# RicherMans/PLDA

Measured on AMD Instinct MI355X. Metric: PLDA LLR trials/sec, higher is better.
Workload: dtype f32; 1 GPU; C2: 100k i-vectors, featdim 200, 5k speakers; 100k x 100k trials, n = 1; fit 10 EM iters; D_eff=200; enrol_models=100000, test_vectors=100000, parallelism=one GPU, score_dtype=f32 (fp64 bias terms, fp32 MFMA contraction), fit_dtype=f64

## Files before the change

### plda_amd/csrc/common.hpp

```cpp
#pragma once

#include <hip/hip_runtime.h>

#include <cstdint>
#include <cstdio>
#include <mutex>
#include <string>
#include <atomic>
#include <vector>

#include "../../include/plda_hip.h"
#include "layout.hpp"

#ifndef PLDA_DIAG
#define PLDA_DIAG 0
#endif

namespace plda {

extern std::atomic<int64_t> g_device_bytes;
extern std::atomic<int64_t> g_device_bytes_peak;
extern std::atomic<int> g_scratch_poison;
extern thread_local hipStream_t g_call_stream;
constexpr size_t POISON_TAIL = (size_t)64 << 10;
// ... 18 lines not shown
}

struct DevBuf {
  void *p = nullptr;
  size_t cap = 0;
  size_t held = 0;
  DevBuf() = default;
  DevBuf(const DevBuf &) = delete;
  DevBuf &operator=(const DevBuf &) = delete;
  ~DevBuf() { release(); }
  hipError_t reserve(size_t bytes) {
    if (bytes <= cap) return hipSuccess;
    release();
    size_t want = bytes + bytes / 8 + 256, total = want + alloc_extra();
    hipError_t e = hipMalloc(&p, total);
    if (e != hipSuccess) { p = nullptr; return e; }
    cap = want; held = total;
    e = alloc_done(p, total);
    if (e != hipSuccess) release();
    return e;
  }
  void release() { free_counted(p, held); p = nullptr; cap = 0; held = 0; }
  template <typename T> T *as() const { return reinterpret_cast<T *>(p); }
};

struct Tmp {
  void *p = nullptr;
  size_t held = 0;
  Tmp() = default;
  Tmp(const Tmp &) = delete;
  Tmp &operator=(const Tmp &) = delete;
  ~Tmp() { free_counted(p, held); }
  hipError_t alloc(size_t bytes) {
    free_counted(p, held); p = nullptr; held = 0;
    const size_t total = (bytes ? bytes : 8) + alloc_extra();
    hipError_t e = hipMalloc(&p, total);
    if (e != hipSuccess) { p = nullptr; return e; }
    held = total;
    e = alloc_done(p, total);
    if (e != hipSuccess) { free_counted(p, held); p = nullptr; held = 0; }
    return e;
  }
  template <typename T> T *as() { return reinterpret_cast<T *>(p); }
};

}

namespace plda { struct HostPipe; }

namespace plda {
constexpr int CS_MAX = 64;
constexpr int CS_NMAX = 4095;
struct CountSet { int G = 0; int32_t vals[CS_MAX] = {}; };
struct Bt4Table { int btM = -1, btN = -1, colwalk = 0; DevBuf tab; int qbase[8] = {}, qlen[8] = {}; uint64_t used = 0; };
}

struct SyrkChunk { const double *rows; int nrows; int pad; double c1, c2; };

struct plda_handle {
  std::recursive_mutex mu;
  int device = 0;
  hipStream_t own_stream = nullptr;
  hipStream_t stream = nullptr;
  std::string err;

  bool fitted = false;
  int Dout = 0, Din = 0;
  std::vector<double> h_mean, h_transform, h_psi, h_offset;
  plda::DevBuf d_mean, d_transform, d_psi, d_offset;
  void *pin_model = nullptr;
  size_t pin_model_cap = 0;

  int64_t fit_K = 0;
  int fit_D = 0;
  plda::DevBuf f_means, f_counts, f_scatter, f_sum, f_W, f_B;
  plda::DevBuf fit_flag;
  plda::DevBuf fit_sort;
  plda::DevBuf fit_offsets;
  plda::DevBuf fit_hist;
  plda::DevBuf fit_roww;
  plda::DevBuf fit_mu;
  plda::DevBuf fit_csum;
  plda::DevBuf em_rows;
  plda::DevBuf em_mats;
  plda::DevBuf grp_pos, grp_uniq;
  double fit_ms[4] = {0, 0, 0, 0};
  hipEvent_t fit_ev[3] = {nullptr, nullptr, nullptr};
  int *fit_dbad = nullptr;
  double fit_t0 = 0.0;

  bool lda_fitted = false;
  int lda_solver = 0, lda_D = 0, lda_rank = 0;
  int64_t lda_K = 0;
  plda::DevBuf l_means, l_priors, l_xbar, l_scalings, l_coef, l_intercept, l_evr;
  plda::DevBuf lda_work;

  plda::HostPipe *hostpipe = nullptr;
  plda::DevBuf hio_O[2];
  int host_variant = 0;

  uint64_t model_epoch = 0;
  struct OneTrial { uint64_t epoch = ~0ull; int n = 0, D = 0; double logterm = 0.0; std::vector<double> c, ivar, ipsi1; } one;

  void *one_host = nullptr, *one_dev = nullptr;
  size_t one_cap = 0;

  plda::DevBuf s_Apk, s_Bpk, s_rbias, s_rscale, s_cbias, s_rpair, s_cpair;
// ... 376 lines not shown
```

### plda_amd/csrc/score.hip

```cpp
#include "common.hpp"
#include <atomic>
#include <chrono>
#include <cstring>

#include <algorithm>

namespace plda {

typedef float f32x4 __attribute__((ext_vector_type(4)));
typedef float f32x16 __attribute__((ext_vector_type(16)));

#define GLOBAL_AS __attribute__((address_space(1)))
#define LDS_AS __attribute__((address_space(3)))

__device__ __forceinline__ void llr_coef(double n, double psi, double &c, double &var) {
  const double den = n * psi + 1.0;
  c = n * psi / den;
  var = 1.0 + psi / den;
}

__global__ void enrol_bias_kernel(const double *__restrict__ U, const int32_t *__restrict__ n_arr,
                                  int n_uniform, const double *__restrict__ psi, int D, int64_t M,
                                  const double *__restrict__ zmean, const double *__restrict__ zstd,
                                  float *__restrict__ rbias, float *__restrict__ rscale) {
  const int lane = threadIdx.x & 63;
  const int64_t row = (int64_t)blockIdx.x * (blockDim.x >> 6) + (threadIdx.x >> 6);
  if (row >= M) return;
  const double n = n_arr ? (double)n_arr[row] : (double)n_uniform;
  const double *u = U + row * (int64_t)D;
  double acc = 0.0;
  for (int d = lane; d < D; d += 64) {
    double c, var;
    const double p = psi[d];
    llr_coef(n, p, c, var);
    const double cu = c * u[d];
    acc += log(var) - log(1.0 + p) + cu * cu / var;
  }
  for (int o = 32; o > 0; o >>= 1) acc += __shfl_xor(acc, o);
  if (lane == 0) {
    double r = -0.5 * acc, sc = 1.0;
    if (zmean && zstd) {
      const double sd = zstd[row];
      if (sd != 0.0) { sc = 1.0 / sd; r = (r - zmean[row]) * sc; }
    }
    rbias[row] = (float)r;
    if (rscale) rscale[row] = (float)sc;
  }
}

__device__ __forceinline__ void count_coef(const double *__restrict__ psi, int D, int n, double *__restrict__ coef ) {
  __shared__ double red[256];
  double acc = 0.0;
  for (int d = threadIdx.x; d < D; d += 256) {
    double c, var;
    const double p = psi[d];
// ... 56 lines not shown
                                                   float *__restrict__ P) {
  __shared__ float tile[32][65];
  const int64_t row0 = (int64_t)blockIdx.x * 64;
  const int k0 = blockIdx.y * 32;
  const int t = threadIdx.x;
  {
    const int c = t & 31;
    const int k = k0 + c;
    const bool second = (MODE == 1 || MODE == 3) && k >= Dp;
    const int d = second ? k - Dp : k;
    const bool dvalid = d < D && k < ((MODE == 1 || MODE == 3) ? 2 * Dp : Dp);
    const double p = dvalid ? psi[d] : 0.0;
#pragma unroll
    for (int pass = 0; pass < 8; ++pass) {
      const int r = (t >> 5) + pass * 8;
      const int64_t row = row0 + r;
      float val = 0.f;
      if (dvalid && row < R) {
        const double x = X[row * (int64_t)D + d];
        if (MODE == 0 || MODE == 1) {
          const double n = n_arr ? (double)n_arr[row] : (double)n_uniform;
          double cc, var;
          llr_coef(n, p, cc, var);
          double v = second ? -0.5 * (1.0 / var - 1.0 / (1.0 + p)) : cc * x / var;
          if (rs) v *= (double)rs[row];
          val = (float)v;
        } else {
          val = (float)(second ? x * x : x);
        }
      }
      tile[c][r] = val;
    }
  }
  __syncthreads();
  {
    const int r = t & 63;
#pragma unroll
    for (int pass = 0; pass < 2; ++pass) {
      const int q = (t >> 6) + pass * 4;
      const int kq = (k0 >> 2) + q;
      if (kq < KQ) {
        f32x4 v;
        v.x = tile[4 * q + 0][r];
        v.y = tile[4 * q + 1][r];
        v.z = tile[4 * q + 2][r];
        v.w = tile[4 * q + 3][r];
        reinterpret_cast<f32x4 *>(P)[(int64_t)kq * Rpad + row0 + r] = v;
      }
    }
  }
}

template <int SIDE, int RW>
__device__ __forceinline__ void prep_side_body(const int block, const double *__restrict__ X, const double *__restrict__ w, const double *__restrict__ Lptr,
                                               int n_uniform, const double *__restrict__ psi, int D, int64_t R, int64_t Rpad, int KQ,
                                               const double *__restrict__ zmean, const double *__restrict__ zstd,
                                               float *__restrict__ P, float *__restrict__ bias, float *__restrict__ rscale,
                                               float2 *__restrict__ pair) {
  constexpr int RPB = 4 * RW;
  __shared__ float tile[2][64][RPB + 1];
  const int lane = threadIdx.x & 63, wave = threadIdx.x >> 6;
  const int64_t row0 = (int64_t)block * RPB;
  const int64_t wrow0 = row0 + wave * RW;
  const int nchunk = (KQ * 4 + 63) >> 6;
  const bool zn = SIDE == 0 && zmean && zstd;
  float rsf[RW];
#pragma unroll
  for (int j = 0; j < RW; ++j) {
    rsf[j] = 1.f;
    if (zn && wrow0 + j < R) { const double sd = zstd[wrow0 + j]; rsf[j] = (float)(sd != 0.0 ? 1.0 / sd : 1.0); }
  }
  constexpr int PF = RW == 16 ? 1 : 4;
  double acc[RW], xc[PF][RW], xn[PF][RW];
#pragma unroll
  for (int j = 0; j < RW; ++j) acc[j] = 0.0;
  auto fetch = [&](int c, double (&x)[RW]) {
    const int d = c * 64 + lane;
#pragma unroll
    for (int j = 0; j < RW; ++j) {
      const int64_t row = wrow0 + j;
      x[j] = (c < nchunk && d < D && row < R) ? X[row * (int64_t)D + d] : 0.0;
    }
  };
  auto chunk = [&](int c, const double (&x)[RW]) {
    const int d = c * 64 + lane;
    const bool dv = d < D;
    const double wd = dv ? w[d] : 0.0;
    double cc = 0.0, var = 1.0;
    if (SIDE == 0 && dv) llr_coef((double)n_uniform, psi[d], cc, var);
    float(*const tl)[RPB + 1] = tile[c & 1];
#pragma unroll
    for (int j = 0; j < RW; ++j) {
      const double xv = x[j];
      float val = 0.f;
      if (dv && wrow0 + j < R) {
        acc[j] += wd * xv * xv;
        if (SIDE == 0) {
          double v = cc * xv / var;
          if (zn) v *= (double)rsf[j];
          val = (float)v;
        } else {
          val = (float)xv;
        }
      }
      tl[lane][wave * RW + j] = val;
    }
    __syncthreads();
    {
      const int r = threadIdx.x % RPB;
#pragma unroll
      for (int pass = 0; pass < RPB / 16; ++pass) {
        const int q = threadIdx.x / RPB + pass * (256 / RPB);
        const int kq = c * 16 + q;
        if (kq < KQ) {
          f32x4 v;
          v.x = tl[4 * q + 0][r];
          v.y = tl[4 * q + 1][r];
          v.z = tl[4 * q + 2][r];
          v.w = tl[4 * q + 3][r];
          reinterpret_cast<f32x4 *>(P)[(int64_t)kq * Rpad + row0 + r] = v;
        }
      }
    }
  };
#pragma unroll
  for (int k = 0; k < PF; ++k) fetch(k, xn[k]);
  for (int c0 = 0; c0 < nchunk; c0 += PF) {
#pragma unroll
    for (int k = 0; k < PF; ++k)
#pragma unroll
      for (int j = 0; j < RW; ++j) xc[k][j] = xn[k][j];
    if (c0 + PF < nchunk) {
#pragma unroll
      for (int k = 0; k < PF; ++k) fetch(c0 + PF + k, xn[k]);
    }
#pragma unroll
    for (int k = 0; k < PF; ++k)
      if (c0 + k < nchunk) chunk(c0 + k, xc[k]);
  }
  const double Lc = SIDE == 0 ? *Lptr : 0.0;
#pragma unroll
  for (int j = 0; j < RW; ++j) {
    double a = acc[j];
    for (int o = 32; o > 0; o >>= 1) a += __shfl_xor(a, o);
    const int64_t row = wrow0 + j;
    if (lane == 0 && row < R) {
      double r = -0.5 * (a + Lc), sc = 1.0;
      if (zn) {
        const double sd = zstd[row];
        if (sd != 0.0) { sc = 1.0 / sd; r = (r - zmean[row]) * sc; }
      }
      bias[row] = (float)r;
      if (SIDE == 0) { rscale[row] = (float)sc; pair[row] = make_float2((float)r, (float)sc); }
      else pair[row] = make_float2(1.f, (float)r);
    }
  }
}

template <int SIDE, int RW>
__global__ __launch_bounds__(256) void prep_side_kernel(const double *__restrict__ X, const double *__restrict__ w, const double *__restrict__ Lptr,
                                                        int n_uniform, const double *__restrict__ psi, int D, int64_t R, int64_t Rpad, int KQ,
                                                        const double *__restrict__ zmean, const double *__restrict__ zstd,
                                                        float *__restrict__ P, float *__restrict__ bias, float *__restrict__ rscale,
                                                        float2 *__restrict__ pair) {
  prep_side_body<SIDE, RW>((int)blockIdx.x, X, w, Lptr, n_uniform, psi, D, R, Rpad, KQ, zmean, zstd, P, bias, rscale, pair);
}
struct PrepSideArgs { const double *X; const double *w; int64_t R, Rpad; float *P; float *bias; float2 *pair; };
__global__ __launch_bounds__(256) void prep_both_kernel(const PrepSideArgs a, const PrepSideArgs b, int blocksA, const double *__restrict__ Lptr, int n_uniform,
                                                        const double *__restrict__ psi, int D, int KQ, const double *__restrict__ zmean,
                                                        const double *__restrict__ zstd, float *__restrict__ rscale) {
  if ((int)blockIdx.x < blocksA)
    prep_side_body<0, 4>((int)blockIdx.x, a.X, a.w, Lptr, n_uniform, psi, D, a.R, a.Rpad, KQ, zmean, zstd, a.P, a.bias, rscale, a.pair);
  else
    prep_side_body<1, 4>((int)blockIdx.x - blocksA, b.X, b.w, Lptr, 0, psi, D, b.R, b.Rpad, KQ, nullptr, nullptr, b.P, b.bias, nullptr, b.pair);
}

struct CountSetDev { int G; int overflow; int32_t vals[CS_MAX]; };

__global__ void count_presence_kernel(const int32_t *__restrict__ n, int64_t M, unsigned char *__restrict__ present ,
                                      int *__restrict__ flags) {
  for (int64_t i = (int64_t)blockIdx.x * blockDim.x + threadIdx.x; i < M; i += (int64_t)gridDim.x * blockDim.x) {
    const int v = n[i];
    if (v >= 1 && v <= CS_NMAX) present[v] = 1;
    else flags[0] = 1;
  }
}

__global__ __launch_bounds__(256) void count_compact_kernel(const unsigned char *__restrict__ present, const int *__restrict__ flags,
                                                            CountSetDev *__restrict__ out) {
  __shared__ unsigned char pr[CS_NMAX + 1];
  for (int i = threadIdx.x; i <= CS_NMAX; i += 256) pr[i] = present[i];
  __syncthreads();
  if (threadIdx.x >= 64) return;
  const int lane = threadIdx.x;
  int cnt = 0;
  for (int k = 0; k < 64; ++k) cnt += pr[lane * 64 + k] ? 1 : 0;
  int incl = cnt;
  for (int o = 1; o < 64; o <<= 1) { const int t = __shfl_up(incl, o); if (lane >= o) incl += t; }
  const int total = __shfl(incl, 63);
  int pos = incl - cnt;
  for (int k = 0; k < 64; ++k)
    if (pr[lane * 64 + k]) { if (pos < CS_MAX) out->vals[pos] = lane * 64 + k; ++pos; }
  if (lane == 0) { out->G = total; out->overflow = (flags[0] != 0 || total > CS_MAX) ? 1 : 0; }
}

constexpr int64_t CS_ONE_WG = 131072;
struct CountSetHost { CountSetDev set; int seq; };
__global__ __launch_bounds__(1024) void count_set_one_wg_kernel(const int32_t *__restrict__ n, int M, int seq, CountSetHost *__restrict__ out ) {
  __shared__ unsigned char pr[CS_NMAX + 1];
  __shared__ int bad;
  for (int i = threadIdx.x; i <= CS_NMAX; i += 1024) pr[i] = 0;
  if (threadIdx.x == 0) bad = 0;
  __syncthreads();
  for (int i0 = 0; i0 < M; i0 += 4096) {
    int v[4];
#pragma unroll
    for (int u = 0; u < 4; ++u) { const int i = i0 + u * 1024 + (int)threadIdx.x; v[u] = i < M ? n[i] : -1; }
#pragma unroll
    for (int u = 0; u < 4; ++u) {
      if (v[u] >= 1 && v[u] <= CS_NMAX) pr[v[u]] = 1;
      else if (i0 + u * 1024 + (int)threadIdx.x < M) bad = 1;
    }
  }
  __syncthreads();
  if (threadIdx.x >= 64) return;
  const int lane = threadIdx.x;
  int cnt = 0;
// ... 687 lines not shown
        unsigned long long *p = dbg + (((size_t)tseq * 16 + 15) * 8 + wave) * 8;
        p[6] = t_e0; p[7] = t_e1;
      }
    }
    ++tseq;
    c_slot = c_slot == 2 ? 0 : c_slot + 1;
    r0 = c_slot == 0 ? q_r0[0] : (c_slot == 1 ? q_r0[1] : q_r0[2]);
    c0 = c_slot == 0 ? q_c0[0] : (c_slot == 1 ? q_c0[1] : q_c0[2]);
    have = (c_slot == 0 ? q_ok[0] : (c_slot == 1 ? q_ok[1] : q_ok[2])) != 0;
  }
  __builtin_amdgcn_s_waitcnt(0x0070);
  if (CLK && threadIdx.x == 0) {
    const unsigned long long c1 = __builtin_amdgcn_s_memtime(), r1 = __builtin_amdgcn_s_memrealtime();
    unsigned long long *p = dbg + 8 + 4 * (size_t)blockIdx.x;
    p[0] = c1 - clk_c0; p[1] = clk_r0; p[2] = r1; p[3] = (unsigned long long)tseq;
    if (blockIdx.x == 0) { dbg[0] = c1 - clk_c0; dbg[1] = r1 - clk_r0; dbg[2] = (unsigned long long)tseq; }
  }
}
#undef BT2_STEP_LAST
#undef BT2_STEP_SECOND
#undef BT2_STEP_FIRST
#undef BT2_STEP_ODD
#undef BT2_XYC
#undef BT2_LOAD
#undef BT2_MFMA8
#undef BT2_MFMA2
#undef BT2_SB

template <typename I = int64_t>
__device__ __host__ inline I bt4_queue_patches(int x, int pM, int pN, int colwalk) {
  if (colwalk) {
    const I rest = (I)pM * (pN % 8);
    return (I)pM * (pN / 8) + (x < rest ? (rest - x + 7) / 8 : 0);
  }
  const I np = (I)pM * pN;
  return x < np ? (np - x + 7) / 8 : 0;
}
template <typename I>
__device__ __host__ inline void bt4_patch(int x, I k, int pM, int pN, int colwalk, int &pm, int &pn) {
  if (colwalk) {
    const I whole = (I)pM * (pN / 8);
    if (k < whole) { pn = x + 8 * (int)(k / pM); pm = (int)(k % pM); }
    else { const int r = pN % 8; const I q = x + 8 * (k - whole); pm = (int)(q / r); pn = (pN / 8) * 8 + (int)(q % r); }
  } else { const I p = x + 8 * k; pm = (int)(p / pN); pn = (int)(p % pN); }
}
#pragma clang diagnostic push
#pragma clang diagnostic ignored "-Wuninitialized"
#pragma clang diagnostic ignored "-Wsometimes-uninitialized"
#pragma clang diagnostic ignored "-Wconditional-uninitialized"
#include "score_bt4.inc"
#pragma clang diagnostic pop
#include "score_bf16x3.inc"

__global__ __launch_bounds__(64) void bt4_table_kernel(int2 *__restrict__ tab, int btM, int btN, int pM, int pN, int colwalk, const Bt4Queues qs) {
  const int x = blockIdx.x, lane = threadIdx.x;
  int off = BT4_QHDR + qs.qbase[x];
  if (lane == 0) tab[x] = make_int2(off, qs.qlen[x]);
  const int64_t nq = bt4_queue_patches(x, pM, pN, colwalk);
  for (int64_t k = 0; k < nq; ++k) {
    int pm, pn;
    bt4_patch(x, k, pM, pN, colwalk, pm, pn);
    const int tm = pm * BPR + lane / BPC, tn = pn * BPC + lane % BPC;
    const bool ok = lane < BPR * BPC && tm < btM && tn < btN;
    const unsigned long long mask = __ballot(ok);
    if (ok) tab[off + __popcll(mask & ((1ull << lane) - 1ull))] = make_int2(tm * 256, tn * 256);
    off += __popcll(mask);
  }
}

static int bt4_schedule(plda_handle *h, int btM, int btN, int KQ, Bt4Table **out) {
  if (!h->bt4_cnt.p) {
    PLDA_HIP(h, h->bt4_cnt.reserve(32 * sizeof(unsigned)));
    PLDA_HIP(h, hipMemsetAsync(h->bt4_cnt.p, 0, 32 * sizeof(unsigned), h->stream));
  }
  const size_t keep = (size_t)128 << 20, bytesA = (size_t)btM * 256 * KQ * 16, bytesB = (size_t)btN * 256 * KQ * 16;
  const int colwalk = h->gemm_variant == 48 ? 0 : h->gemm_variant == 49 ? 1 : (bytesA <= keep && bytesB > keep) ? 1 : 0;
  Bt4Table *lru = &h->bt4_tabs[0];
  for (auto &t : h->bt4_tabs) {
    if (t.btM == btM && t.btN == btN && t.colwalk == colwalk) { t.used = ++h->bt4_clock; *out = &t; return PLDA_OK; }
    if (t.used < lru->used) lru = &t;
  }
  Bt4Table &t = *lru;
  const int pM = (int)ceil_div(btM, BPR), pN = (int)ceil_div(btN, BPC);
  int64_t total = 0;
  Bt4Queues qs;
  for (int x = 0; x < 8; ++x) {
    t.qbase[x] = (int)total;
    const int64_t nq = bt4_queue_patches(x, pM, pN, colwalk);
    for (int64_t k = 0; k < nq; ++k) {
      int pm, pn;
      bt4_patch(x, k, pM, pN, colwalk, pm, pn);
      total += (int64_t)std::min(BPR, btM - pm * BPR) * std::min(BPC, btN - pn * BPC);
    }
    t.qlen[x] = (int)total - t.qbase[x];
    qs.qbase[x] = t.qbase[x]; qs.qlen[x] = t.qlen[x];
  }
  t.btM = t.btN = -1;
  PLDA_HIP(h, t.tab.reserve((size_t)(total + BT4_QHDR + 1) * sizeof(int2))   );
  bt4_table_kernel<<<8, 64, 0, h->stream>>>(t.tab.as<int2>(), btM, btN, pM, pN, colwalk, qs);
  PLDA_LAUNCH_CHECK(h);
  t.btM = btM; t.btN = btN; t.colwalk = colwalk; t.used = ++h->bt4_clock;
  *out = &t;
  return PLDA_OK;
}

__global__ void znorm_finalize_kernel(const float *__restrict__ shift, const double *__restrict__ colsum,
                                      const double *__restrict__ colsq, int64_t M, double invN,
                                      double *__restrict__ out_mean, double *__restrict__ out_std) {
  const int64_t j = (int64_t)blockIdx.x * blockDim.x + threadIdx.x;
  if (j >= M) return;
  const double m1 = colsum[j] * invN;
  double var = colsq[j] * invN - m1 * m1;
  if (var < 0.0) var = 0.0;
  out_mean[j] = (double)shift[j] + m1;
  out_std[j] = sqrt(var);
}

__global__ void pilot_shift_kernel(const double *__restrict__ colsum, int64_t M, double invN,
                                   float *__restrict__ shift) {
  const int64_t j = (int64_t)blockIdx.x * blockDim.x + threadIdx.x;
  if (j < M) shift[j] = (float)(colsum[j] * invN);
}

__global__ void score_pairs_kernel(const double *__restrict__ U, const int32_t *__restrict__ n_enrol,
                                   const double *__restrict__ V, const int64_t *__restrict__ e_idx,
                                   const int64_t *__restrict__ t_idx, int64_t P,
                                   const double *__restrict__ psi, int D,
                                   const double *__restrict__ zmean, const double *__restrict__ zstd,
                                   double *__restrict__ out) {
  const int lane = threadIdx.x & 63;
  const int64_t p = (int64_t)blockIdx.x * (blockDim.x >> 6) + (threadIdx.x >> 6);
  if (p >= P) return;
  const int64_t e = e_idx[p], t = t_idx[p];
  const double n = (double)n_enrol[e];
  const double *u = U + e * (int64_t)D, *v = V + t * (int64_t)D;
  double acc = 0.0;
  for (int d = lane; d < D; d += 64) {
    double c, var;
    const double ps = psi[d];
    llr_coef(n, ps, c, var);
    const double diff = v[d] - c * u[d];
    acc += (log(var) + diff * diff / var) - (log(1.0 + ps) + v[d] * v[d] / (1.0 + ps));
  }
  for (int o = 32; o > 0; o >>= 1) acc += __shfl_xor(acc, o);
  if (lane == 0) {
    double s = -0.5 * acc;
    if (zmean && zstd && zstd[e] != 0.0) s = (s - zmean[e]) / zstd[e];
    out[p] = s;
  }
}

constexpr int64_t PAIRS_TAB_MIN = 16384;
__global__ void pairs_validate_kernel(const int64_t *__restrict__ e, const int64_t *__restrict__ t, int64_t P, int64_t M, int64_t Nt,
                                      unsigned long long *__restrict__ first_bad) {
// ... 146 lines not shown
    if (doA && doB && few(op.Mpad) && few(op.Npad)) {
      const PrepBucketArgs a{dU, dn, M, op.Mpad, h->s_Apk.as<float>(), h->s_rbias.as<float>(), h->s_rscale.as<float>(), h->s_rpair.as<float2>(),
                             dV, Nt, op.Npad, h->s_Bpk.as<float>(), h->s_cbias.as<float>(), h->s_cpair.as<float2>()};
      prep_buckets_both_kernel<<<(unsigned)((op.Mpad + op.Npad) / 16), 256, 0, h->stream>>>(a, (int)(op.Mpad / 16), *cs, coefG, h->d_psi.as<double>(), D,
                                                                                           KQm, KQx, dzmean, dzstd);
      PLDA_LAUNCH_CHECK(h);
      return PLDA_OK;
    }
    if (doA) {
      if (few(op.Mpad))
        prep_enrol_buckets_kernel<4><<<(unsigned)(op.Mpad / 16), 256, 0, h->stream>>>(
            dU, dn, *cs, coefG, h->d_psi.as<double>(), D, M, op.Mpad, KQm, KQx, dzmean, dzstd, h->s_Apk.as<float>(),
            h->s_rbias.as<float>(), h->s_rscale.as<float>(), h->s_rpair.as<float2>());
      else
        prep_enrol_buckets_kernel<16><<<(unsigned)(op.Mpad / 64), 256, 0, h->stream>>>(
            dU, dn, *cs, coefG, h->d_psi.as<double>(), D, M, op.Mpad, KQm, KQx, dzmean, dzstd, h->s_Apk.as<float>(),
            h->s_rbias.as<float>(), h->s_rscale.as<float>(), h->s_rpair.as<float2>());
    }
    if (doB) {
      if (few(op.Npad)) {
        prep_side_kernel<1, 4><<<(unsigned)(op.Npad / 16), 256, 0, h->stream>>>(
            dV, coefG + D, coefG + 2 * D, 0, h->d_psi.as<double>(), D, Nt, op.Npad, KQm, nullptr, nullptr, h->s_Bpk.as<float>(),
            h->s_cbias.as<float>(), nullptr, h->s_cpair.as<float2>());
        prep_test_buckets_kernel<4><<<(unsigned)(op.Npad / 16), 256, 0, h->stream>>>(dV, coefG, G, D, Nt, op.Npad, KQm, KQx, h->s_Bpk.as<float>());
      } else {
        prep_side_kernel<1, 16><<<(unsigned)(op.Npad / 64), 256, 0, h->stream>>>(
            dV, coefG + D, coefG + 2 * D, 0, h->d_psi.as<double>(), D, Nt, op.Npad, KQm, nullptr, nullptr, h->s_Bpk.as<float>(),
            h->s_cbias.as<float>(), nullptr, h->s_cpair.as<float2>());
        prep_test_buckets_kernel<16><<<(unsigned)(op.Npad / 64), 256, 0, h->stream>>>(dV, coefG, G, D, Nt, op.Npad, KQm, KQx, h->s_Bpk.as<float>());
      }
    }
    PLDA_LAUNCH_CHECK(h);
    return PLDA_OK;
  }
  const double *psi = h->d_psi.as<double>();
  const bool zn = dzmean && dzstd;
  const int wpb = 4;
  if (op.mixed) {
    if (doA)
      enrol_bias_kernel<<<(unsigned)ceil_div(M, wpb), wpb * 64, 0, h->stream>>>(
          dU, dn, n_uniform, psi, D, M, dzmean, dzstd, h->s_rbias.as<float>(), h->s_rscale.as<float>());
    if (doB) PLDA_HIP(h, hipMemsetAsync(h->s_cbias.p, 0, (size_t)op.Npad * 4, h->stream));
  } else {
    PLDA_HIP(h, h->coef_cache.reserve((size_t)(2 * D + 1) * 8));
    double *coef = h->coef_cache.as<double>();
    if (!(h->ucoef_ptr == coef && h->ucoef_epoch == h->model_epoch && h->ucoef_n == n_uniform && h->ucoef_D == D)) {
      uniform_coef_kernel<<<1, 256, 0, h->stream>>>(psi, D, n_uniform, coef);
      h->gcoef_ptr = nullptr;
      h->ucoef_ptr = coef; h->ucoef_epoch = h->model_epoch; h->ucoef_n = n_uniform; h->ucoef_D = D;
    }
    if (h->prep_variant != 1) {
      auto few_rows = [&](int64_t rpad) { return h->prep_variant == 3 || (h->prep_variant != 2 && rpad <= 32768); };
#define PREP_SIDE(SIDE_, RW_, RPAD_, ...) prep_side_kernel<SIDE_, RW_><<<(unsigned)((RPAD_) / (4 * RW_)), 256, 0, h->stream>>>(__VA_ARGS__)
      if (doA && doB && few_rows(op.Mpad) && few_rows(op.Npad)) {
        const PrepSideArgs a{dU, coef, M, op.Mpad, h->s_Apk.as<float>(), h->s_rbias.as<float>(), h->s_rpair.as<float2>()};
        const PrepSideArgs b{dV, coef + D, Nt, op.Npad, h->s_Bpk.as<float>(), h->s_cbias.as<float>(), h->s_cpair.as<float2>()};
        prep_both_kernel<<<(unsigned)((op.Mpad + op.Npad) / 16), 256, 0, h->stream>>>(a, b, (int)(op.Mpad / 16), coef + 2 * D, n_uniform, psi, D, op.KQ,
                                                                                     dzmean, dzstd, h->s_rscale.as<float>());
        PLDA_LAUNCH_CHECK(h);
        return PLDA_OK;
      }
      if (doA) {
        if (few_rows(op.Mpad))
          PREP_SIDE(0, 4, op.Mpad, dU, coef, coef + 2 * D, n_uniform, psi, D, M, op.Mpad, op.KQ, dzmean, dzstd, h->s_Apk.as<float>(),
                    h->s_rbias.as<float>(), h->s_rscale.as<float>(), h->s_rpair.as<float2>());
        else
          PREP_SIDE(0, 16, op.Mpad, dU, coef, coef + 2 * D, n_uniform, psi, D, M, op.Mpad, op.KQ, dzmean, dzstd, h->s_Apk.as<float>(),
                    h->s_rbias.as<float>(), h->s_rscale.as<float>(), h->s_rpair.as<float2>());
      }
      if (doB) {
        if (few_rows(op.Npad))
          PREP_SIDE(1, 4, op.Npad, dV, coef + D, coef + 2 * D, 0, psi, D, Nt, op.Npad, op.KQ, nullptr, nullptr, h->s_Bpk.as<float>(),
                    h->s_cbias.as<float>(), nullptr, h->s_cpair.as<float2>());
        else
          PREP_SIDE(1, 16, op.Npad, dV, coef + D, coef + 2 * D, 0, psi, D, Nt, op.Npad, op.KQ, nullptr, nullptr, h->s_Bpk.as<float>(),
                    h->s_cbias.as<float>(), nullptr, h->s_cpair.as<float2>());
      }
#undef PREP_SIDE
      PLDA_LAUNCH_CHECK(h);
      return PLDA_OK;
    }
    if (doA)
      weighted_sq_bias_kernel<<<(unsigned)ceil_div(M, wpb), wpb * 64, 0, h->stream>>>(
          dU, coef, 1.0, coef + 2 * D, D, M, dzmean, dzstd, h->s_rbias.as<float>(), h->s_rscale.as<float>());
    if (doB)
      weighted_sq_bias_kernel<<<(unsigned)ceil_div(Nt, wpb), wpb * 64, 0, h->stream>>>(
          dV, coef + D, 0.0, coef + 2 * D, D, Nt, nullptr, nullptr, h->s_cbias.as<float>(), nullptr);
  }
  {
    const int64_t ma = doA ? M : 0, nb = doB ? Nt : 0;
    bias_pairs_kernel<<<(unsigned)ceil_div(std::max(ma, nb), 256), 256, 0, h->stream>>>(
        h->s_rbias.as<float>(), h->s_rscale.as<float>(), ma, h->s_cbias.as<float>(), nb,
        h->s_rpair.as<float2>(), h->s_cpair.as<float2>());
  }
  PLDA_LAUNCH_CHECK(h);
  const float *rs = zn ? h->s_rscale.as<float>() : nullptr;
  const dim3 ga((unsigned)(op.Mpad / 64), (unsigned)ceil_div(op.Kg, 32));
  const dim3 gb((unsigned)(op.Npad / 64), (unsigned)ceil_div(op.Kg, 32));
  if (op.mixed) {
    if (doA)
      pack_kernel<1><<<ga, 256, 0, h->stream>>>(dU, dn, n_uniform, psi, rs, D, Dp, M, op.Mpad,
                                                op.KQ, h->s_Apk.as<float>());
    if (doB)
      pack_kernel<3><<<gb, 256, 0, h->stream>>>(dV, nullptr, 0, psi, nullptr, D, Dp, Nt, op.Npad,
                                                op.KQ, h->s_Bpk.as<float>());
  } else {
    if (doA)
      pack_kernel<0><<<ga, 256, 0, h->stream>>>(dU, dn, n_uniform, psi, rs, D, Dp, M, op.Mpad,
                                                op.KQ, h->s_Apk.as<float>());
    if (doB)
      pack_kernel<2><<<gb, 256, 0, h->stream>>>(dV, nullptr, 0, psi, nullptr, D, Dp, Nt, op.Npad,
// ... 33 lines not shown
    split_bf16x3_kernel<<<dim3((unsigned)(op.Npad / 256), (unsigned)KO), 256, 0, h->stream>>>(h->s_Bpk.as<f32x4>(), op.Npad, op.KQ, h->s_B16.as<f32x4>());
    static DeviceOnce once;
    if (once.needed(h->device)) {
      const void *fns[] = {reinterpret_cast<const void *>(&trials_gemm_bf16x3_kernel<0>),
#if PLDA_DIAG
                           reinterpret_cast<const void *>(&trials_gemm_bf16x3_kernel<4>), reinterpret_cast<const void *>(&trials_gemm_bf16x3_kernel<8>),
                           reinterpret_cast<const void *>(&trials_gemm_bf16x3_kernel<12>), reinterpret_cast<const void *>(&trials_gemm_bf16x3_kernel<16>),
#endif
      };
      for (const void *f : fns) PLDA_HIP(h, hipFuncSetAttribute(f, hipFuncAttributeMaxDynamicSharedMemorySize, B3_LDS));
      once.done(h->device);
    }
    const int b3M = (int)ceil_div(M, 256), b3N = (int)ceil_div(Nt, 128);
    const int pM = (int)ceil_div(b3M, B3_PR), pN = (int)ceil_div(b3N, B3_PC);
    const size_t keep3 = (size_t)128 << 20, bytesA3 = (size_t)3 * KO * op.Mpad * 16, bytesB3 = (size_t)3 * KO * op.Npad * 16;
    const int colwalk3 = h->gemm_variant == 48 ? 0 : h->gemm_variant == 49 ? 1 : (bytesA3 <= keep3 && bytesB3 > keep3) ? 1 : 0;
    h->last_kernel = "trials_gemm_bf16x3_kernel";
#define B3L(MODE_)                                                                                                                      \
  trials_gemm_bf16x3_kernel<MODE_><<<256, 512, B3_LDS, h->stream>>>(h->s_A16.as<f32x4>(), h->s_B16.as<f32x4>(), (unsigned)op.Mpad, (unsigned)op.Npad,  \
                                                                    nsteps, h->s_rbias.as<float>(), h->s_rscale.as<float>(), h->s_cbias.as<float>(), dout, \
                                                                    ld, M, Nt, b3M, b3N, pM, pN, colwalk3, h->timeline.as<unsigned long long>())
#if PLDA_DIAG
    if (h->gemm_variant == 63) {
      PLDA_HIP(h, h->timeline.reserve(TIMELINE_WORDS * 8));
      B3L(16);
      h->timeline_valid = true;
    } else if (h->gemm_variant == 54) B3L(4);
    else if (h->gemm_variant == 58) B3L(8);
    else if (h->gemm_variant == 62) B3L(12);
    else
#endif
      B3L(0);
#undef B3L
    PLDA_LAUNCH_CHECK(h);
    if (ev1) PLDA_HIP(h, hipEventRecord(ev1, h->stream));
    return PLDA_OK;
  }
  const int btM = (int)ceil_div(M, 256), btN = (int)(op.Npad / 256);
  const int64_t tiles = (int64_t)btM * btN;
  const bool patches_full = (double)tiles >= 0.85 * (double)(round_up(btM, BPR) * round_up(btN, BPC));
  const bool old_rule = h->gemm_variant == 50;
  const bool big = EPI == 0 && tiles >= (old_rule ? 1024 : 1700);
  const bool big2 = EPI == 0 && (old_rule ? tiles >= 1024 : (tiles >= 1700 || (tiles >= 512 && patches_full)));
  const bool fits4g = (int64_t)(op.KQ + 8) * op.Mpad * 16 < (1ll << 32) && (int64_t)(op.KQ + 8) * op.Npad * 16 < (1ll << 32);
  const bool use_bt2 = EPI == 0 && fits4g && ld < (1ll << 22) &&
                       ((h->gemm_variant >= 30 && h->gemm_variant <= 37) || ((h->gemm_variant == 0 || old_rule) && big2));
  {
    const int nsteps = op.KQ >> 1, nst = (nsteps + 3) >> 2;
    const bool use_bt4 = EPI == 0 && fits4g && ld < (1ll << 22) && nst >= 3 && M < (1ll << 31) && Nt < (1ll << 31) &&
                         (h->gemm_variant == 40 || h->gemm_variant == 41 || h->gemm_variant == 48 || h->gemm_variant == 49 || (h->gemm_variant >= 44 && h->gemm_variant <= 47) || ((h->gemm_variant == 0 || old_rule) && big));
    if (use_bt4) {
      const int sbase = nsteps / nst, fs = sbase + (nsteps - sbase * nst > 0 ? 1 : 0);
      h->last_kernel = "trials_gemm_bt4_kernel";
      Bt4Table *tb = nullptr;
      PLDA_TRY(bt4_schedule(h, btM, btN, op.KQ, &tb));
      const int rag_m = (M & 255) != 0, rag_n = (Nt & 255) != 0;
      const int fslots = (rag_m || rag_n) ? btM + btN : 0;
      PLDA_HIP(h, h->bt4_fringe.reserve(std::max<size_t>((size_t)fslots * 65536 * 4, 256)));
      if (!h->bt4_attr_set) {
        const void *fns[] = {reinterpret_cast<const void *>(&trials_gemm_bt4_kernel<3, 0>), reinterpret_cast<const void *>(&trials_gemm_bt4_kernel<4, 0>),
#if PLDA_DIAG
                             reinterpret_cast<const void *>(&trials_gemm_bt4_kernel<3, 1>), reinterpret_cast<const void *>(&trials_gemm_bt4_kernel<4, 1>),
                             reinterpret_cast<const void *>(&trials_gemm_bt4_kernel<4, 4>), reinterpret_cast<const void *>(&trials_gemm_bt4_kernel<4, 8>),
                             reinterpret_cast<const void *>(&trials_gemm_bt4_kernel<4, 12>), reinterpret_cast<const void *>(&trials_gemm_bt4_kernel<4, 16>),
                             reinterpret_cast<const void *>(&trials_gemm_bt4_kernel<3, 16>),
#endif
        };
        for (const void *f : fns) PLDA_HIP(h, hipFuncSetAttribute(f, hipFuncAttributeMaxDynamicSharedMemorySize, BT4_LDS));
        h->bt4_attr_set = true;
      }
#define BT4L(FS_, MODE_, DBG_)                                                                            \
  trials_gemm_bt4_kernel<FS_, MODE_><<<256, 256, BT4_LDS, h->stream>>>(                                   \
      h->s_Apk.as<f32x4>(), h->s_Bpk.as<f32x4>(), (unsigned)op.Mpad, (unsigned)op.Npad, op.KQ,            \
      h->s_rpair.as<float2>(), h->s_cpair.as<float2>(), dout, ld, (int)M, (int)Nt, h->bt4_fringe.as<float>(), tb->tab.as<int2>(), h->bt4_cnt.as<unsigned>(), DBG_)
#if PLDA_DIAG
      if (h->gemm_variant == 41) {
        PLDA_HIP(h, h->timeline.reserve(TIMELINE_WORDS * 8));
        PLDA_HIP(h, hipMemsetAsync(h->timeline.p, 0, TIMELINE_WORDS * 8, h->stream));
        if (fs == 3) BT4L(3, 1, h->timeline.as<unsigned long long>());
        else BT4L(4, 1, h->timeline.as<unsigned long long>());
        h->timeline_valid = true;
      } else if (h->gemm_variant == 47) {
        PLDA_HIP(h, h->timeline.reserve(TIMELINE_WORDS * 8));
        if (fs == 3) BT4L(3, 16, h->timeline.as<unsigned long long>());
        else BT4L(4, 16, h->timeline.as<unsigned long long>());
        h->timeline_valid = true;
      } else if (h->gemm_variant >= 44 && h->gemm_variant <= 46 && fs == 4) {
        if (h->gemm_variant == 44) BT4L(4, 4, nullptr);
        else if (h->gemm_variant == 45) BT4L(4, 8, nullptr);
        else BT4L(4, 12, nullptr);
      } else
#endif
      if (fs == 3) {
        BT4L(3, 0, nullptr);
      } else {
        BT4L(4, 0, nullptr);
      }
#undef BT4L
      if (fslots)
        fringe_copy_kernel<<<(unsigned)(fslots * 8), 256, 0, h->stream>>>(h->bt4_fringe.as<float>(), dout, ld, (int)M, (int)Nt, btM, btN, rag_m, rag_n);
      PLDA_LAUNCH_CHECK(h);
      if (ev1) PLDA_HIP(h, hipEventRecord(ev1, h->stream));
      return PLDA_OK;
    }
  }
  if (use_bt2) {
    h->last_kernel = "trials_gemm_bt2_kernel";
    const int pM = (int)ceil_div(btM, BPR), pN = (int)ceil_div(btN, BPC);
    if (!h->bt2_attr_set) {
      const void *fns[] = {reinterpret_cast<const void *>(&trials_gemm_bt2_kernel<0>), reinterpret_cast<const void *>(&trials_gemm_bt2_kernel<2>),
#if PLDA_DIAG
                           reinterpret_cast<const void *>(&trials_gemm_bt2_kernel<1>), reinterpret_cast<const void *>(&trials_gemm_bt2_kernel<3>),
                           reinterpret_cast<const void *>(&trials_gemm_bt2_kernel<4>), reinterpret_cast<const void *>(&trials_gemm_bt2_kernel<8>),
                           reinterpret_cast<const void *>(&trials_gemm_bt2_kernel<12>), reinterpret_cast<const void *>(&trials_gemm_bt2_kernel<16>),
#endif
      };
      for (const void *f : fns) PLDA_HIP(h, hipFuncSetAttribute(f, hipFuncAttributeMaxDynamicSharedMemorySize, BT2_LDS));
      h->bt2_attr_set = true;
    }
#define BT2L(MODE_, DBG_)                                                                                 \
  trials_gemm_bt2_kernel<MODE_><<<256, 512, BT2_LDS, h->stream>>>(                                        \
      h->s_Apk.as<f32x4>(), h->s_Bpk.as<f32x4>(), (unsigned)op.Mpad, (unsigned)op.Npad, op.KQ,            \
      h->s_rpair.as<float2>(), h->s_cpair.as<float2>(), dout, ld, M, Nt, btM, btN, pN, pM * pN, DBG_)
#if PLDA_DIAG
    if (h->gemm_variant == 31 || h->gemm_variant == 33) {
      PLDA_HIP(h, h->timeline.reserve(TIMELINE_WORDS * 8));
      PLDA_HIP(h, hipMemsetAsync(h->timeline.p, 0, TIMELINE_WORDS * 8, h->stream));
      if (h->gemm_variant == 31) BT2L(1, h->timeline.as<unsigned long long>());
      else BT2L(3, h->timeline.as<unsigned long long>());
      h->timeline_valid = true;
    } else if (h->gemm_variant == 37) {
      PLDA_HIP(h, h->timeline.reserve(TIMELINE_WORDS * 8));
      BT2L(16, h->timeline.as<unsigned long long>());
      h->timeline_valid = true;
    } else if (h->gemm_variant == 34) {
      BT2L(4, nullptr);
    } else if (h->gemm_variant == 35) {
      BT2L(8, nullptr);
    } else if (h->gemm_variant == 36) {
      BT2L(12, nullptr);
    } else
#endif
    if (h->gemm_variant == 32) {
      BT2L(2, nullptr);
    } else {
      BT2L(0, nullptr);
    }
#undef BT2L
    PLDA_LAUNCH_CHECK(h);
    if (ev1) PLDA_HIP(h, hipEventRecord(ev1, h->stream));
    return PLDA_OK;
  }
#define TG(NKQ_, EPI_, MINW_, ABL_)                                                                     \
// ... 468 lines not shown
```

Baseline: 358.2 billion trials/s.

## Shift ragged edge tiles inward instead of using fringe scratch copy

For ragged M/N with even sizes and at least 256 rows/cols, the last 256-tile is shifted to start at M-256 (or Nt-256), so it overlaps the previous tile and writes directly to output. This removes the fringe scratch buffer and the separate fringe_copy kernel for these cases, at the cost of recomputing some overlapping rows and columns. The combined prep_both kernel is also templated, so large padded sizes can use the RW=16 variant instead of separate per-side launches. For 100k, which is not a multiple of 256, the shift path is active.

```diff
diff --git a/plda_amd/csrc/common.hpp b/plda_amd/csrc/common.hpp
--- a/plda_amd/csrc/common.hpp
+++ b/plda_amd/csrc/common.hpp
@@ -94,7 +94,7 @@
 constexpr int CS_MAX = 64;
 constexpr int CS_NMAX = 4095;
 struct CountSet { int G = 0; int32_t vals[CS_MAX] = {}; };
-struct Bt4Table { int btM = -1, btN = -1, colwalk = 0; DevBuf tab; int qbase[8] = {}, qlen[8] = {}; uint64_t used = 0; };
+struct Bt4Table { int btM = -1, btN = -1, colwalk = 0, rmax = 0, cmax = 0, scratch = 0; DevBuf tab; int qbase[8] = {}, qlen[8] = {}; uint64_t used = 0; };
 }
 
 struct SyrkChunk { const double *rows; int nrows; int pad; double c1, c2; };
diff --git a/plda_amd/csrc/score.hip b/plda_amd/csrc/score.hip
--- a/plda_amd/csrc/score.hip
+++ b/plda_amd/csrc/score.hip
@@ -1,6 +1,7 @@
 #include "common.hpp"
 #include <atomic>
 #include <chrono>
+#include <climits>
 #include <cstring>
 
 #include <algorithm>
@@ -163,13 +164,12 @@
 }
 
 template <int SIDE, int RW>
-__device__ __forceinline__ void prep_side_body(const int block, const double *__restrict__ X, const double *__restrict__ w, const double *__restrict__ Lptr,
+__device__ __forceinline__ void prep_side_core(const int block, const double *__restrict__ X, const double *__restrict__ w, const double *__restrict__ Lptr,
                                                int n_uniform, const double *__restrict__ psi, int D, int64_t R, int64_t Rpad, int KQ,
                                                const double *__restrict__ zmean, const double *__restrict__ zstd,
                                                float *__restrict__ P, float *__restrict__ bias, float *__restrict__ rscale,
-                                               float2 *__restrict__ pair) {
+                                               float2 *__restrict__ pair, float (*tile)[64][4 * RW + 1]) {
   constexpr int RPB = 4 * RW;
-  __shared__ float tile[2][64][RPB + 1];
   const int lane = threadIdx.x & 63, wave = threadIdx.x >> 6;
   const int64_t row0 = (int64_t)block * RPB;
   const int64_t wrow0 = row0 + wave * RW;
@@ -269,6 +269,16 @@
 }
 
 template <int SIDE, int RW>
+__device__ __forceinline__ void prep_side_body(const int block, const double *__restrict__ X, const double *__restrict__ w, const double *__restrict__ Lptr,
+                                               int n_uniform, const double *__restrict__ psi, int D, int64_t R, int64_t Rpad, int KQ,
+                                               const double *__restrict__ zmean, const double *__restrict__ zstd,
+                                               float *__restrict__ P, float *__restrict__ bias, float *__restrict__ rscale,
+                                               float2 *__restrict__ pair) {
+  __shared__ float tile[2][64][4 * RW + 1];
+  prep_side_core<SIDE, RW>(block, X, w, Lptr, n_uniform, psi, D, R, Rpad, KQ, zmean, zstd, P, bias, rscale, pair, tile);
+}
+
+template <int SIDE, int RW>
 __global__ __launch_bounds__(256) void prep_side_kernel(const double *__restrict__ X, const double *__restrict__ w, const double *__restrict__ Lptr,
                                                         int n_uniform, const double *__restrict__ psi, int D, int64_t R, int64_t Rpad, int KQ,
                                                         const double *__restrict__ zmean, const double *__restrict__ zstd,
@@ -277,13 +287,15 @@
   prep_side_body<SIDE, RW>((int)blockIdx.x, X, w, Lptr, n_uniform, psi, D, R, Rpad, KQ, zmean, zstd, P, bias, rscale, pair);
 }
 struct PrepSideArgs { const double *X; const double *w; int64_t R, Rpad; float *P; float *bias; float2 *pair; };
+template <int RW>
 __global__ __launch_bounds__(256) void prep_both_kernel(const PrepSideArgs a, const PrepSideArgs b, int blocksA, const double *__restrict__ Lptr, int n_uniform,
                                                         const double *__restrict__ psi, int D, int KQ, const double *__restrict__ zmean,
                                                         const double *__restrict__ zstd, float *__restrict__ rscale) {
+  __shared__ float tile[2][64][4 * RW + 1];
   if ((int)blockIdx.x < blocksA)
-    prep_side_body<0, 4>((int)blockIdx.x, a.X, a.w, Lptr, n_uniform, psi, D, a.R, a.Rpad, KQ, zmean, zstd, a.P, a.bias, rscale, a.pair);
+    prep_side_core<0, RW>((int)blockIdx.x, a.X, a.w, Lptr, n_uniform, psi, D, a.R, a.Rpad, KQ, zmean, zstd, a.P, a.bias, rscale, a.pair, tile);
   else
-    prep_side_body<1, 4>((int)blockIdx.x - blocksA, b.X, b.w, Lptr, 0, psi, D, b.R, b.Rpad, KQ, nullptr, nullptr, b.P, b.bias, nullptr, b.pair);
+    prep_side_core<1, RW>((int)blockIdx.x - blocksA, b.X, b.w, Lptr, 0, psi, D, b.R, b.Rpad, KQ, nullptr, nullptr, b.P, b.bias, nullptr, b.pair, tile);
 }
 
 struct CountSetDev { int G; int overflow; int32_t vals[CS_MAX]; };
@@ -1077,7 +1089,7 @@
 #pragma clang diagnostic pop
 #include "score_bf16x3.inc"
 
-__global__ __launch_bounds__(64) void bt4_table_kernel(int2 *__restrict__ tab, int btM, int btN, int pM, int pN, int colwalk, const Bt4Queues qs) {
+__global__ __launch_bounds__(64) void bt4_table_kernel(int2 *__restrict__ tab, int btM, int btN, int pM, int pN, int colwalk, int rmax, int cmax, int scratch, const Bt4Queues qs) {
   const int x = blockIdx.x, lane = threadIdx.x;
   int off = BT4_QHDR + qs.qbase[x];
   if (lane == 0) tab[x] = make_int2(off, qs.qlen[x]);
@@ -1088,12 +1100,15 @@
     const int tm = pm * BPR + lane / BPC, tn = pn * BPC + lane % BPC;
     const bool ok = lane < BPR * BPC && tm < btM && tn < btN;
     const unsigned long long mask = __ballot(ok);
-    if (ok) tab[off + __popcll(mask & ((1ull << lane) - 1ull))] = make_int2(tm * 256, tn * 256);
+    if (ok) {
+      const bool in_scratch = ((scratch & 1) && tm == btM - 1) || ((scratch & 2) && tn == btN - 1);
+      tab[off + __popcll(mask & ((1ull << lane) - 1ull))] = in_scratch ? make_int2(tm * 256, tn * 256) : make_int2(min(tm * 256, rmax), min(tn * 256, cmax));
+    }
     off += __popcll(mask);
   }
 }
 
-static int bt4_schedule(plda_handle *h, int btM, int btN, int KQ, Bt4Table **out) {
+static int bt4_schedule(plda_handle *h, int btM, int btN, int KQ, int rmax, int cmax, int scratch, Bt4Table **out) {
   if (!h->bt4_cnt.p) {
     PLDA_HIP(h, h->bt4_cnt.reserve(32 * sizeof(unsigned)));
     PLDA_HIP(h, hipMemsetAsync(h->bt4_cnt.p, 0, 32 * sizeof(unsigned), h->stream));
@@ -1102,7 +1117,7 @@
   const int colwalk = h->gemm_variant == 48 ? 0 : h->gemm_variant == 49 ? 1 : (bytesA <= keep && bytesB > keep) ? 1 : 0;
   Bt4Table *lru = &h->bt4_tabs[0];
   for (auto &t : h->bt4_tabs) {
-    if (t.btM == btM && t.btN == btN && t.colwalk == colwalk) { t.used = ++h->bt4_clock; *out = &t; return PLDA_OK; }
+    if (t.btM == btM && t.btN == btN && t.colwalk == colwalk && t.rmax == rmax && t.cmax == cmax && t.scratch == scratch) { t.used = ++h->bt4_clock; *out = &t; return PLDA_OK; }
     if (t.used < lru->used) lru = &t;
   }
   Bt4Table &t = *lru;
@@ -1122,9 +1137,9 @@
   }
   t.btM = t.btN = -1;
   PLDA_HIP(h, t.tab.reserve((size_t)(total + BT4_QHDR + 1) * sizeof(int2))   );
-  bt4_table_kernel<<<8, 64, 0, h->stream>>>(t.tab.as<int2>(), btM, btN, pM, pN, colwalk, qs);
+  bt4_table_kernel<<<8, 64, 0, h->stream>>>(t.tab.as<int2>(), btM, btN, pM, pN, colwalk, rmax, cmax, scratch, qs);
   PLDA_LAUNCH_CHECK(h);
-  t.btM = btM; t.btN = btN; t.colwalk = colwalk; t.used = ++h->bt4_clock;
+  t.btM = btM; t.btN = btN; t.colwalk = colwalk; t.rmax = rmax; t.cmax = cmax; t.scratch = scratch; t.used = ++h->bt4_clock;
   *out = &t;
   return PLDA_OK;
 }
@@ -1377,11 +1392,15 @@
     if (h->prep_variant != 1) {
       auto few_rows = [&](int64_t rpad) { return h->prep_variant == 3 || (h->prep_variant != 2 && rpad <= 32768); };
 #define PREP_SIDE(SIDE_, RW_, RPAD_, ...) prep_side_kernel<SIDE_, RW_><<<(unsigned)((RPAD_) / (4 * RW_)), 256, 0, h->stream>>>(__VA_ARGS__)
-      if (doA && doB && few_rows(op.Mpad) && few_rows(op.Npad)) {
+      if (doA && doB && few_rows(op.Mpad) == few_rows(op.Npad)) {
         const PrepSideArgs a{dU, coef, M, op.Mpad, h->s_Apk.as<float>(), h->s_rbias.as<float>(), h->s_rpair.as<float2>()};
         const PrepSideArgs b{dV, coef + D, Nt, op.Npad, h->s_Bpk.as<float>(), h->s_cbias.as<float>(), h->s_cpair.as<float2>()};
-        prep_both_kernel<<<(unsigned)((op.Mpad + op.Npad) / 16), 256, 0, h->stream>>>(a, b, (int)(op.Mpad / 16), coef + 2 * D, n_uniform, psi, D, op.KQ,
-                                                                                     dzmean, dzstd, h->s_rscale.as<float>());
+        if (few_rows(op.Mpad))
+          prep_both_kernel<4><<<(unsigned)((op.Mpad + op.Npad) / 16), 256, 0, h->stream>>>(a, b, (int)(op.Mpad / 16), coef + 2 * D, n_uniform, psi, D, op.KQ,
+                                                                                          dzmean, dzstd, h->s_rscale.as<float>());
+        else
+          prep_both_kernel<16><<<(unsigned)((op.Mpad + op.Npad) / 64), 256, 0, h->stream>>>(a, b, (int)(op.Mpad / 64), coef + 2 * D, n_uniform, psi, D, op.KQ,
+                                                                                           dzmean, dzstd, h->s_rscale.as<float>());
         PLDA_LAUNCH_CHECK(h);
         return PLDA_OK;
       }
@@ -1521,11 +1540,15 @@
     if (use_bt4) {
       const int sbase = nsteps / nst, fs = sbase + (nsteps - sbase * nst > 0 ? 1 : 0);
       h->last_kernel = "trials_gemm_bt4_kernel";
+      const int rag_m = (M & 255) != 0, rag_n = (Nt & 255) != 0;
+      const bool can_shift = M >= 256 && Nt >= 256;
+      const int sh_m = rag_m && can_shift && (M & 1) == 0, sh_n = rag_n && can_shift && (Nt & 1) == 0;
+      const int fb_m = rag_m && !sh_m, fb_n = rag_n && !sh_n;
       Bt4Table *tb = nullptr;
-      PLDA_TRY(bt4_schedule(h, btM, btN, op.KQ, &tb));
-      const int rag_m = (M & 255) != 0, rag_n = (Nt & 255) != 0;
-      const int fslots = (rag_m || rag_n) ? btM + btN : 0;
-      PLDA_HIP(h, h->bt4_fringe.reserve(std::max<size_t>((size_t)fslots * 65536 * 4, 256)));
+      PLDA_TRY(bt4_schedule(h, btM, btN, op.KQ, sh_m ? (int)M - 256 : INT_MAX, sh_n ? (int)Nt - 256 : INT_MAX, fb_m | (fb_n << 1), &tb));
+      const int Mk = sh_m ? btM * 256 : (int)M, Nk = sh_n ? btN * 256 : (int)Nt;
+      const int fslots = (fb_m || fb_n) ? btM + btN : 0;
+      if (fslots) PLDA_HIP(h, h->bt4_fringe.reserve((size_t)fslots * 65536 * 4));
       if (!h->bt4_attr_set) {
         const void *fns[] = {reinterpret_cast<const void *>(&trials_gemm_bt4_kernel<3, 0>), reinterpret_cast<const void *>(&trials_gemm_bt4_kernel<4, 0>),
 #if PLDA_DIAG
@@ -1541,7 +1564,7 @@
 #define BT4L(FS_, MODE_, DBG_)                                                                            \
   trials_gemm_bt4_kernel<FS_, MODE_><<<256, 256, BT4_LDS, h->stream>>>(                                   \
       h->s_Apk.as<f32x4>(), h->s_Bpk.as<f32x4>(), (unsigned)op.Mpad, (unsigned)op.Npad, op.KQ,            \
-      h->s_rpair.as<float2>(), h->s_cpair.as<float2>(), dout, ld, (int)M, (int)Nt, h->bt4_fringe.as<float>(), tb->tab.as<int2>(), h->bt4_cnt.as<unsigned>(), DBG_)
+      h->s_rpair.as<float2>(), h->s_cpair.as<float2>(), dout, ld, Mk, Nk, h->bt4_fringe.as<float>(), tb->tab.as<int2>(), h->bt4_cnt.as<unsigned>(), DBG_)
 #if PLDA_DIAG
       if (h->gemm_variant == 41) {
         PLDA_HIP(h, h->timeline.reserve(TIMELINE_WORDS * 8));
@@ -1567,7 +1590,7 @@
       }
 #undef BT4L
       if (fslots)
-        fringe_copy_kernel<<<(unsigned)(fslots * 8), 256, 0, h->stream>>>(h->bt4_fringe.as<float>(), dout, ld, (int)M, (int)Nt, btM, btN, rag_m, rag_n);
+        fringe_copy_kernel<<<(unsigned)(fslots * 8), 256, 0, h->stream>>>(h->bt4_fringe.as<float>(), dout, ld, (int)M, (int)Nt, btM, btN, fb_m, fb_n);
       PLDA_LAUNCH_CHECK(h);
       if (ev1) PLDA_HIP(h, hipEventRecord(ev1, h->stream));
       return PLDA_OK;
```

Result: no change. 359.8 billion trials/s (median of 6 runs) (+0.5%).
